# KhutornoyYaroslav/vcm-ts

Measured on AMD Instinct MI355X. Metric: encoded frames/sec at 1920x1080 GOP-32, higher is better.
Workload: dtype f32 (fp16x3 split-MFMA, fp32 accumulate)

## Files before the change

include/dcvc_hip.h:

```cpp
#ifndef DCVC_HIP_H
#define DCVC_HIP_H

#include <stdint.h>

#ifdef __cplusplus
extern "C" {
#endif

#define DCVC_OK 0
#define DCVC_E_ARG (-1)
#define DCVC_E_LAUNCH (-2)
#define DCVC_E_RANGE (-3)

#define DCVC_STATUS_ACT_SATURATED 1

#define DCVC_MAX_SEG 3

#define DCVC_PREC_FP32 0
#define DCVC_PREC_FP16X3 1

typedef struct {
    const float *ptr;
    int32_t C;
    int32_t cs;
} dcvc_seg;

typedef struct {
    dcvc_seg seg[DCVC_MAX_SEG];
    int32_t nseg;
    int32_t N, Hin, Win;
    int32_t in_act;
    float in_slope;
    const float *wpack;
    const float *bpack;
    int32_t ks;
    int32_t stride;
    int32_t Cout;
    int32_t Cout_pad;
    float *out;
    int32_t out_cs;
    int32_t out_act;
    float out_slope;
    int32_t pixel_shuffle;
    const float *res;
    int32_t res_cs;
    const float *res_gate;
    const float *res2;
    int32_t res2_cs;
    int32_t precision;
    int32_t *status;
    float *chan_partial;
    int32_t tile_row0;
    int32_t tile_rows;
    int32_t pair_taps;
} dcvc_conv_args;

int32_t dcvc_conv_tile_rows(int32_t ks, int32_t stride);

int32_t dcvc_conv_chan_partial_parts(int32_t ks, int32_t stride, int32_t Hout, int32_t Wout);
int dcvc_channel_mean_finish(const float *chan_partial, int32_t parts, int32_t row_stride, float *mean, int32_t N,
                             int32_t C, int32_t HW, void *stream);

int64_t dcvc_conv_pack_size(int32_t Cout, int32_t ks, int32_t nseg, const int32_t *seg_C, int32_t *cout_pad);

int dcvc_conv_pack_weights(const float *w, const float *b, int32_t Cout, int32_t ks, int32_t nseg,
                           const int32_t *seg_C, int32_t pixel_shuffle, int32_t precision, float *wpack,
                           float *bpack);

int64_t dcvc_conv_pack_size_paired(int32_t Cout, int32_t Cin, int32_t *cout_pad);
int dcvc_conv_pack_weights_paired(const float *w, const float *b, int32_t Cout, int32_t Cin, float *wpack, float *bpack);

int dcvc_conv2d(const dcvc_conv_args *a, void *stream);

int64_t dcvc_conv_small_pack_bytes(int32_t Cout, int32_t ks, int32_t nseg, const int32_t *seg_C);
int dcvc_conv_small_pack_weights(const float *w, const float *b, int32_t Cout, int32_t ks, int32_t nseg,
                                 const int32_t *seg_C, void *wpack, float *bpack);
int dcvc_conv2d_small(const dcvc_conv_args *a, void *stream);

int64_t dcvc_conv_k32_pack_bytes(int32_t Cout, int32_t ks, int32_t nseg, const int32_t *seg_C, int32_t *cout_pad);
int dcvc_conv_k32_pack_weights(const float *w, const float *b, int32_t Cout, int32_t ks, int32_t nseg,
                               const int32_t *seg_C, int32_t pixel_shuffle, void *wpack, float *bpack);
int dcvc_conv2d_k32(const dcvc_conv_args *a, void *stream);
int dcvc_conv_k32_set_waves(int32_t waves);

int dcvc_warp(const float *src, int32_t src_cs, const float *flow, int32_t flow_cs, float *out, int32_t out_cs,
              int32_t N, int32_t H, int32_t W, int32_t C, void *stream);
int dcvc_up2(const float *src, int32_t src_cs, float *out, int32_t out_cs, float *out2, int32_t out2_cs,
             int32_t N, int32_t H, int32_t W, int32_t C, float scale, void *stream);
int dcvc_down2(const float *src, int32_t src_cs, float *out, int32_t out_cs, int32_t N, int32_t H, int32_t W,
               int32_t C, float scale, int32_t avgpool_order, void *stream);
int dcvc_maxpool2(const float *src, int32_t src_cs, float *out, int32_t out_cs, int32_t N, int32_t H, int32_t W,
                  int32_t C, void *stream);
int dcvc_copy_channels(const float *src, int32_t src_cs, float *out, int32_t out_cs, int64_t npix, int32_t C,
                       void *stream);
int dcvc_nchw_to_nhwc(const float *src, float *out, int32_t out_cs, int32_t N, int32_t C, int32_t H, int32_t W,
                      void *stream);
int dcvc_nhwc_to_nchw(const float *src, int32_t src_cs, float *out, int32_t N, int32_t C, int32_t H, int32_t W,
                      int32_t clamp01, void *stream);

int dcvc_channel_mean(const float *src, int32_t src_cs, float *mean, float *scratch, int32_t N, int32_t HW,
                      int32_t C, void *stream);
int dcvc_se_gate(const float *mean, const float *w1, const float *w2, float *gate, int32_t N, int32_t C,
                 int32_t Cr, void *stream);

int dcvc_scale_channels(const float *src, int32_t src_cs, float *out, int32_t out_cs, const float *q_basic,
                        const float *q_scale, int32_t mode, int32_t N, int32_t HW, int32_t C, void *stream);
int dcvc_round_symbols(const float *z, int32_t z_cs, float *z_hat, int32_t zh_cs, int32_t *sym, int32_t N,
                       int32_t H, int32_t W, int32_t C, void *stream);
int dcvc_symbols_to_nhwc(const int32_t *sym, float *out, int32_t out_cs, int32_t N, int32_t H, int32_t W,
                         int32_t C, void *stream);

typedef struct {
    const float *y;
    int32_t y_cs;
    const float *fusion;
    int32_t fusion_cs;
    const float *spatial;
    int32_t spatial_cs;
    float *params;
    int32_t params_cs;
    float *y_hat;
    float *y_q;
    float *y_res;
    float *scales_hat;
    int32_t *sym;
// ... 36 lines not shown
```

vcm_ts_amd/csrc/conv_mfma.hip:

```cpp
#include <hip/hip_runtime.h>
#include <stdint.h>
#include <stdlib.h>
#include <string.h>
#include <vector>

#include "dcvc_hip.h"

typedef float f32x16 __attribute__((ext_vector_type(16)));
typedef float f32x4 __attribute__((ext_vector_type(4)));
typedef _Float16 f16x8 __attribute__((ext_vector_type(8)));
typedef _Float16 f16x4 __attribute__((ext_vector_type(4)));

namespace {

constexpr int KC = 16;
constexpr int LDK = 20;

constexpr float ACT_SCALE = 8.f;
constexpr float WGT_SCALE = 64.f;
constexpr float F16_MAX = 65504.f;

struct ConvK {
    const float *seg_ptr[DCVC_MAX_SEG];
    int seg_C[DCVC_MAX_SEG];
    int seg_cs[DCVC_MAX_SEG];
    int nseg;
    int Hin, Win, Hout, Wout;
    int in_act;
    float in_slope;
    const float *wpack;
    const float *bpack;
    int Cout, Cout_pad;
    float *out;
    int out_cs;
    int out_act;
    float out_slope;
    int ps;
    const float *res;
    int res_cs;
    const float *res_gate;
    const float *res2;
    int res2_cs;
    int vec_epi;
    int *status;
    float *chan_partial;
    int ntx;
    int ty0, nty;
    int band_rows;
};

constexpr float ACT_LIMIT = 65504.f / 8.f;

__device__ __forceinline__ float act(float v, float slope) { return v > 0.f ? v : v * slope; }

inline long dev_env_long(const char *name, long dflt) {
    const char *dev = getenv("DCVC_DEV");
    if (!dev || strcmp(dev, "1") != 0) return dflt;
    const char *v = getenv(name);
    return v ? atol(v) : dflt;
}


template <int KS, int S, int RPW, int NT, bool SPLIT, bool PAIR = false>
__global__ __launch_bounds__(256, 2) void conv_mfma(const ConvK a) {
    static_assert(!PAIR || (KS == 7 && S == 1 && SPLIT), "tap pairing is built for the 7x7 split-fp16 layers");
    constexpr int BH = 4 * RPW, BW = 32, BN = 32 * NT;
    constexpr int PH = (BH - 1) * S + KS, PW = (BW - 1) * S + KS, PAD = KS / 2;
    constexpr int T = PAIR ? KS * 4 : KS * KS;
    constexpr int TPS = PAIR ? 4 : (KS == 3 && S == 1) ? 9 : KS;
    constexpr int NST = T / TPS;
    constexpr int EPI_LD = BN + 4;
    constexpr int LDS_MAIN = PH * PW * LDK + TPS * 4 * BN * 4, LDS_EPI = 4 * 32 * EPI_LD, LDS_RED = 4 * BN;
    __shared__ __attribute__((aligned(16))) float lds[LDS_MAIN > LDS_EPI + LDS_RED ? LDS_MAIN : LDS_EPI + LDS_RED];
    float *patch = lds;
    float *wl = lds + PH * PW * LDK;

    const int tid = threadIdx.x, lane = tid & 63, wave = tid >> 6;
    const int nbn = a.Cout_pad / BN;
    const int nb = blockIdx.x % nbn, tx = blockIdx.x / nbn;
    if (tx >= a.ntx) return;
    const int ty = blockIdx.y + a.ty0;
    const int x0 = tx * BW, y0 = ty * BH, n0 = nb * BN, img = blockIdx.z;

    f32x16 acc[RPW][NT];
#pragma unroll
    for (int m = 0; m < RPW; ++m)
#pragma unroll
        for (int n = 0; n < NT; ++n)
#pragma unroll
            for (int r = 0; r < 16; ++r) acc[m][n][r] = 0.f;

    const int a_base = ((wave * RPW * S) * PW + (lane & 31) * S) * LDK + (lane >> 5) * 4;
    const int b_base = ((lane >> 5) * BN + (lane & 31)) * 4;

    constexpr int NP = (PH * PW * 4 + 255) / 256, NW = (TPS * 4 * BN + 255) / 256;
    f32x4 rp[NP], rw[NW];
    struct Cursor {
        int s, c0, cg, st;
    };
    auto advance = [&](Cursor &k) {
        if (++k.st == NST) {
            k.st = 0;
            ++k.cg;
            k.c0 += KC;
            if (k.c0 >= a.seg_C[k.s]) {
                ++k.s;
                k.c0 = 0;
            }
        }
    };
    int poff[NP];
    unsigned inpic = 0;
#pragma unroll
    for (int u = 0; u < NP; ++u) {
        const int i = tid + u * 256;
        const int p = i >> 2;
        const int py = p / PW, px = p - py * PW + (PAIR ? (i & 3) >> 1 : 0);
        const int gy = y0 * S - PAD + py, gx = x0 * S - PAD + px;
        const bool ok = i < PH * PW * 4 && gy >= 0 && gy < a.Hin && gx >= 0 && gx < a.Win;
        poff[u] = ok ? gy * a.Win + gx : 0;
        inpic |= (ok ? 1u : 0u) << u;
    }
    auto load_patch = [&](const Cursor &k) {
        const int C = a.seg_C[k.s], cs = a.seg_cs[k.s];
        const float *sp = a.seg_ptr[k.s] + (size_t)img * a.Hin * a.Win * cs;
        const int c = PAIR ? (tid & 1) * 4 : k.c0 + (tid & 3) * 4;
        const int cc = c < C ? c : 0;
#pragma unroll
        for (int u = 0; u < NP; ++u) rp[u] = *(const f32x4 *)(sp + (size_t)poff[u] * cs + cc);
    };
    auto store_patch = [&](const Cursor &k) {
        const int C = a.seg_C[k.s];
#pragma unroll
        for (int u = 0; u < NP; ++u) {
            const int i = tid + u * 256;
            if (i < PH * PW * 4) {
                const int c = PAIR ? (i & 1) * 4 : k.c0 + (i & 3) * 4;
                f32x4 v = ((inpic >> u) & 1u) && c < C ? rp[u] : (f32x4){0.f, 0.f, 0.f, 0.f};
                if (c + 3 >= C) {
                    if (c + 1 >= C) v[1] = 0.f;
                    if (c + 2 >= C) v[2] = 0.f;
                    v[3] = 0.f;
                }
                if (a.in_act) {
                    v[0] = act(v[0], a.in_slope);
                    v[1] = act(v[1], a.in_slope);
                    v[2] = act(v[2], a.in_slope);
                    v[3] = act(v[3], a.in_slope);
                }
                if (!SPLIT) {
                    *(f32x4 *)&patch[(i >> 2) * LDK + (i & 3) * 4] = v;
                } else {
                    f32x4 sv = v * ACT_SCALE;
#pragma unroll
                    for (int e = 0; e < 4; ++e) sv[e] = __builtin_amdgcn_fmed3f(sv[e], -F16_MAX, F16_MAX);
                    const f16x4 hi = __builtin_convertvector(sv, f16x4);
                    const f16x4 lo = __builtin_convertvector(sv - __builtin_convertvector(hi, f32x4), f16x4);
                    _Float16 *rec = (_Float16 *)&patch[(i >> 2) * LDK];
                    *(f16x4 *)&rec[(i & 3) * 4] = hi;
                    *(f16x4 *)&rec[16 + (i & 3) * 4] = lo;
                }
            }
        }
    };
    auto load_w = [&](const Cursor &k) {
        const float *wsrc = a.wpack + ((size_t)(k.cg * T + k.st * TPS) * 4) * a.Cout_pad * 4 + (size_t)n0 * 4;
#pragma unroll
        for (int u = 0; u < NW; ++u) {
            const int i = tid + u * 256;
            const int row = i / BN, col = i - row * BN;
            if (i < TPS * 4 * BN) rw[u] = *(const f32x4 *)(wsrc + ((size_t)row * a.Cout_pad + col) * 4);
        }
    };
    auto store_w = [&]() {
#pragma unroll
        for (int u = 0; u < NW; ++u) {
            const int i = tid + u * 256;
            if (i < TPS * 4 * BN) *(f32x4 *)&wl[i * 4] = rw[u];
        }
    };

    Cursor cur = {0, 0, 0, 0};
    load_patch(cur);
    load_w(cur);
    while (cur.s < a.nseg) {
        __syncthreads();
        if (cur.st == 0) store_patch(cur);
        store_w();
        __syncthreads();
        Cursor nxt = cur;
        advance(nxt);
        if (nxt.s < a.nseg) {
            if (nxt.st == 0) load_patch(nxt);
            load_w(nxt);
        }
        const int a_st = (TPS == T) ? 0 : cur.st * PW * LDK;
#pragma unroll
        for (int tt = 0; tt < TPS; ++tt) {
            const int ky = (TPS == T) ? tt / KS : 0, kx = PAIR ? 2 * tt : (TPS == T) ? tt % KS : tt;
            if (!SPLIT) {
#pragma unroll
                for (int k2 = 0; k2 < 2; ++k2) {
                    f32x4 af[RPW], bf[NT];
#pragma unroll
                    for (int m = 0; m < RPW; ++m)
                        af[m] = *(const f32x4 *)&patch[a_base + a_st + ((m * S + ky) * PW + kx) * LDK + k2 * 8];
#pragma unroll
                    for (int n = 0; n < NT; ++n)
                        bf[n] = *(const f32x4 *)&wl[b_base + ((tt * 4 + k2 * 2) * BN + n * 32) * 4];
#pragma unroll
                    for (int j = 0; j < 4; ++j)
#pragma unroll
                        for (int m = 0; m < RPW; ++m)
#pragma unroll
                            for (int n = 0; n < NT; ++n)
                                acc[m][n] = __builtin_amdgcn_mfma_f32_32x32x2f32(af[m][j], bf[n][j], acc[m][n], 0, 0, 0);
                }
            } else {
                f16x8 ah[RPW], al[RPW], bh[NT], bl[NT];
#pragma unroll
                for (int m = 0; m < RPW; ++m) {
                    const float *rec = &patch[a_base + a_st + ((m * S + ky) * PW + kx) * LDK];
                    ah[m] = *(const f16x8 *)rec;
                    al[m] = *(const f16x8 *)(rec + 8);
                }
#pragma unroll
                for (int n = 0; n < NT; ++n) {
                    bh[n] = *(const f16x8 *)&wl[b_base + ((tt * 4) * BN + n * 32) * 4];
                    bl[n] = *(const f16x8 *)&wl[b_base + ((tt * 4 + 2) * BN + n * 32) * 4];
                }
#pragma unroll
                for (int m = 0; m < RPW; ++m)
#pragma unroll
                    for (int n = 0; n < NT; ++n) {
                        acc[m][n] = __builtin_amdgcn_mfma_f32_32x32x16_f16(ah[m], bh[n], acc[m][n], 0, 0, 0);
                        acc[m][n] = __builtin_amdgcn_mfma_f32_32x32x16_f16(ah[m], bl[n], acc[m][n], 0, 0, 0);
                        acc[m][n] = __builtin_amdgcn_mfma_f32_32x32x16_f16(al[m], bh[n], acc[m][n], 0, 0, 0);
                    }
            }
        }
        cur = nxt;
    }

    const int col = lane & 31, hh = lane >> 5;
    const int Cq = a.Cout >> 2;
    const int Cfin = a.ps ? Cq : a.Cout;
    const int Ho = a.ps ? a.Hout * 2 : a.Hout, Wo = a.ps ? a.Wout * 2 : a.Wout;
    const float inv_scale = SPLIT ? 1.f / (ACT_SCALE * WGT_SCALE) : 1.f;
    float vmax = 0.f;
    if (a.vec_epi) {
        constexpr int LPP = BN / 4, PPI = 64 / LPP, NIT = 32 / PPI;
        float *epi = lds + wave * 32 * EPI_LD;
        const int c4 = (lane % LPP) * 4, pl = lane / LPP;
        const int ch = n0 + c4;
        const bool ch_ok = ch < a.Cout;
        int dy = 0, dx = 0, cf = ch;
        if (a.ps) {
            const int sub = ch / Cq;
            cf = ch - sub * Cq;
            dy = sub >> 1;
            dx = sub & 1;
        }
        f32x4 bias = {0.f, 0.f, 0.f, 0.f}, gate = {1.f, 1.f, 1.f, 1.f};
        if (ch_ok) {
            bias = *(const f32x4 *)&a.bpack[ch];
            if (a.res_gate) gate = *(const f32x4 *)&a.res_gate[(size_t)img * Cfin + cf];
        }
        __syncthreads();
        size_t pix[RPW][NIT];
        bool ok[RPW][NIT];
        f32x4 rv[RPW][NIT], rv2[RPW][NIT];
        f32x4 csum = {0.f, 0.f, 0.f, 0.f};
#pragma unroll
        for (int m = 0; m < RPW; ++m) {
            const int oy = y0 + wave * RPW + m;
#pragma unroll
            for (int it = 0; it < NIT; ++it) {
// ... 69 lines not shown
        return;
    }
#pragma unroll
    for (int m = 0; m < RPW; ++m) {
        const int oy = y0 + wave * RPW + m;
        if (oy >= a.Hout) continue;
#pragma unroll
        for (int n = 0; n < NT; ++n) {
            const int ch = n0 + n * 32 + col;
            if (ch >= a.Cout) continue;
            const float bias = a.bpack[ch];
            int dy = 0, dx = 0, cf = ch;
            if (a.ps) {
                const int sub = ch / Cq;
                cf = ch - sub * Cq;
                dy = sub >> 1;
                dx = sub & 1;
            }
            const float gate = a.res_gate ? a.res_gate[(size_t)img * Cfin + cf] : 1.f;
            float rv[16], rv2[16];
#pragma unroll
            for (int r = 0; r < 16; ++r) {
                const int ox = x0 + (r & 3) + 8 * (r >> 2) + 4 * hh;
                const size_t pix = a.ps ? ((size_t)(img * Ho + 2 * oy + dy) * Wo + 2 * ox + dx)
                                        : ((size_t)(img * Ho + oy) * Wo + ox);
                rv[r] = (a.res && ox < a.Wout) ? a.res[pix * a.res_cs + cf] : 0.f;
                rv2[r] = (a.res2 && ox < a.Wout) ? a.res2[pix * a.res2_cs + cf] : 0.f;
            }
#pragma unroll
            for (int r = 0; r < 16; ++r) {
                const int ox = x0 + (r & 3) + 8 * (r >> 2) + 4 * hh;
                if (ox >= a.Wout) continue;
                float v = acc[m][n][r] * inv_scale + bias;
                if (a.out_act == 1) v = act(v, a.out_slope);
                else if (a.out_act == 2) v = fminf(fmaxf(v, 0.f), 1.f);
                const size_t pix = a.ps ? ((size_t)(img * Ho + 2 * oy + dy) * Wo + 2 * ox + dx)
                                        : ((size_t)(img * Ho + oy) * Wo + ox);
                if (a.out_act == 3) {
                    const float mk = rv2[r] > 0.f ? 1.f : a.out_slope;
                    v = a.res ? __builtin_fmaf(v, mk, rv[r]) : v * mk;
                } else {
                    if (a.res) v = a.res_gate ? __builtin_fmaf(rv[r], gate, v) : v + rv[r];
                    if (a.res2) v = rv2[r] + v;
                }
                if (a.status) vmax = fmaxf(vmax, fabsf(v));
                a.out[pix * a.out_cs + cf] = v;
            }
        }
    }
    if (a.status && !(vmax <= ACT_LIMIT)) atomicOr(a.status, DCVC_STATUS_ACT_SATURATED);
}


template <int KS, int S, int RPW, int NT, bool PAIR = false>
int launch(ConvK &k, int N, hipStream_t st, int precision) {
    constexpr int BH = 4 * RPW, BN = 32 * NT;
    k.ntx = (k.Wout + 31) / 32;
    static const bool xcd_pad = dev_env_long("DCVC_XCD_PAD", 0) != 0;
    unsigned gx = (unsigned)(k.ntx * (k.Cout_pad / BN));
    if (xcd_pad && gx >= 8) gx = (gx + 7) & ~7u;
    k.nty = (k.Hout + BH - 1) / BH;
    if (k.ty0 < 0 || k.ty0 >= k.nty) return DCVC_E_ARG;
    const int rows = k.band_rows > 0 ? (k.band_rows < k.nty - k.ty0 ? k.band_rows : k.nty - k.ty0) : k.nty;
    dim3 grid(gx, (unsigned)rows, (unsigned)N);
    if (PAIR)
        hipLaunchKernelGGL((conv_mfma<KS, S, RPW, NT, true, PAIR>), grid, dim3(256), 0, st, k);
    else if (precision == DCVC_PREC_FP16X3)
        hipLaunchKernelGGL((conv_mfma<KS, S, RPW, NT, true>), grid, dim3(256), 0, st, k);
    else
        hipLaunchKernelGGL((conv_mfma<KS, S, RPW, NT, false>), grid, dim3(256), 0, st, k);
    return hipGetLastError() == hipSuccess ? DCVC_OK : DCVC_E_LAUNCH;
}

inline int round_up(int v, int m) { return (v + m - 1) / m * m; }

}

extern "C" int64_t dcvc_conv_pack_size(int32_t Cout, int32_t ks, int32_t nseg, const int32_t *seg_C, int32_t *cout_pad) {
    if (Cout <= 0 || nseg <= 0 || nseg > DCVC_MAX_SEG || (ks != 1 && ks != 3 && ks != 7)) return DCVC_E_ARG;
    int chunks = 0;
    for (int s = 0; s < nseg; ++s) chunks += (seg_C[s] + KC - 1) / KC;
    const int cp = round_up(Cout, 32);
    if (cout_pad) *cout_pad = cp;
    return (int64_t)chunks * ks * ks * 4 * cp * 4;
}

extern "C" int dcvc_conv_pack_weights(const float *w, const float *b, int32_t Cout, int32_t ks, int32_t nseg,
                                      const int32_t *seg_C, int32_t pixel_shuffle, int32_t precision, float *wpack,
                                      float *bpack) {
    if (precision != DCVC_PREC_FP32 && precision != DCVC_PREC_FP16X3) return DCVC_E_ARG;
    int32_t cp = 0;
    const int64_t total = dcvc_conv_pack_size(Cout, ks, nseg, seg_C, &cp);
    if (total < 0 || (pixel_shuffle && (Cout & 3))) return DCVC_E_ARG;
    const int T = ks * ks;
    int Cin = 0;
    for (int s = 0; s < nseg; ++s) Cin += seg_C[s];
    memset(wpack, 0, (size_t)total * sizeof(float));
    memset(bpack, 0, (size_t)cp * sizeof(float));
    const int Cq = Cout / 4;
    int cg = 0, cin0 = 0;
    for (int s = 0; s < nseg; ++s) {
        for (int c0 = 0; c0 < seg_C[s]; c0 += KC, ++cg) {
            for (int t = 0; t < T; ++t)
                for (int kq = 0; kq < 4; ++kq)
                    for (int j = 0; j < 4; ++j) {
                        const int c = c0 + kq * 4 + j;
                        if (c >= seg_C[s]) continue;
                        for (int n = 0; n < Cout; ++n) {
                            const int np = pixel_shuffle ? (n & 3) * Cq + (n >> 2) : n;
                            const float v = w[((size_t)n * Cin + cin0 + c) * T + t];
                            if (precision == DCVC_PREC_FP32) {
                                wpack[((((size_t)cg * T + t) * 4 + kq) * cp + np) * 4 + j] = v;
                            } else {
                                const int cc = kq * 4 + j, h = cc >> 3, jj = cc & 7;
                                float sv = v * WGT_SCALE;
                                sv = sv > F16_MAX ? F16_MAX : (sv < -F16_MAX ? -F16_MAX : sv);
                                const _Float16 hi = (_Float16)sv, lo = (_Float16)(sv - (float)hi);
                                _Float16 *base = (_Float16 *)wpack;
// ... 6 lines not shown
        cin0 += seg_C[s];
    }
    for (int n = 0; n < Cout; ++n) {
        const int np = pixel_shuffle ? (n & 3) * Cq + (n >> 2) : n;
        bpack[np] = b ? b[n] : 0.f;
    }
    return DCVC_OK;
}

extern "C" int64_t dcvc_conv_pack_size_paired(int32_t Cout, int32_t Cin, int32_t *cout_pad) {
    if (Cout <= 0 || Cin <= 0 || Cin > 8) return DCVC_E_ARG;
    const int cp = round_up(Cout, 32);
    if (cout_pad) *cout_pad = cp;
    return (int64_t)7 * 4 * 4 * cp * 4;
}

extern "C" int dcvc_conv_pack_weights_paired(const float *w, const float *b, int32_t Cout, int32_t Cin, float *wpack, float *bpack) {
    int32_t cp = 0;
    const int64_t total = dcvc_conv_pack_size_paired(Cout, Cin, &cp);
    if (total < 0 || !w || !wpack || !bpack) return DCVC_E_ARG;
    memset(wpack, 0, (size_t)total * sizeof(float));
    memset(bpack, 0, (size_t)cp * sizeof(float));
    _Float16 *base = (_Float16 *)wpack;
    bool clamped = false;
    for (int ky = 0; ky < 7; ++ky)
        for (int kx = 0; kx < 7; ++kx) {
            const int step = ky * 4 + (kx >> 1), h = kx & 1;
            for (int c = 0; c < Cin; ++c)
                for (int n = 0; n < Cout; ++n) {
                    float sv = w[((size_t)n * Cin + c) * 49 + ky * 7 + kx] * WGT_SCALE;
                    if (!(fabsf(sv) <= F16_MAX)) {
                        clamped = true;
                        sv = sv > 0.f ? F16_MAX : -F16_MAX;
                    }
                    const _Float16 hi = (_Float16)sv, lo = (_Float16)(sv - (float)hi);
                    base[(((size_t)step * 4 + h) * cp + n) * 8 + c] = hi;
                    base[(((size_t)step * 4 + 2 + h) * cp + n) * 8 + c] = lo;
                }
        }
    for (int n = 0; n < Cout; ++n) bpack[n] = b ? b[n] : 0.f;
    return clamped ? DCVC_E_RANGE : DCVC_OK;
}

static int tile_rows(int ks, int stride) { return stride == 2 ? 4 : 8; }

extern "C" int32_t dcvc_conv_tile_rows(int32_t ks, int32_t stride) { return tile_rows(ks, stride); }

extern "C" int32_t dcvc_conv_chan_partial_parts(int32_t ks, int32_t stride, int32_t Hout, int32_t Wout) {
    if (Hout <= 0 || Wout <= 0 || (stride != 1 && stride != 2)) return DCVC_E_ARG;
    const int bh = tile_rows(ks, stride);
    return ((Wout + 31) / 32) * ((Hout + bh - 1) / bh);
}

extern "C" int dcvc_conv2d(const dcvc_conv_args *a, void *stream) {
    if (!a || a->nseg < 1 || a->nseg > DCVC_MAX_SEG || !a->out || !a->wpack || !a->bpack) return DCVC_E_ARG;
    if (a->stride != 1 && a->stride != 2) return DCVC_E_ARG;
    if (a->precision != DCVC_PREC_FP32 && a->precision != DCVC_PREC_FP16X3) return DCVC_E_ARG;
    if (a->Cout_pad % 32 || a->Cout > a->Cout_pad || (a->pixel_shuffle && (a->Cout & 3))) return DCVC_E_ARG;
    if (a->out_act < 0 || a->out_act > 3) return DCVC_E_ARG;
    if (a->out_act == 3 && (!a->res2 || a->res_gate || a->chan_partial || a->pixel_shuffle)) return DCVC_E_ARG;
    ConvK k;
    memset(&k, 0, sizeof(k));
    for (int s = 0; s < a->nseg; ++s) {
        if (!a->seg[s].ptr || (a->seg[s].cs & 3) || a->seg[s].cs < round_up(a->seg[s].C, 4) ||
            ((uintptr_t)a->seg[s].ptr & 15))
            return DCVC_E_ARG;
        k.seg_ptr[s] = a->seg[s].ptr;
        k.seg_C[s] = a->seg[s].C;
        k.seg_cs[s] = a->seg[s].cs;
    }
    k.nseg = a->nseg;
    k.Hin = a->Hin;
    k.Win = a->Win;
    const int pad = a->ks / 2;
    k.Hout = (a->Hin + 2 * pad - a->ks) / a->stride + 1;
    k.Wout = (a->Win + 2 * pad - a->ks) / a->stride + 1;
    k.in_act = a->in_act;
    k.in_slope = a->in_slope;
    k.wpack = a->wpack;
    k.bpack = a->bpack;
    k.Cout = a->Cout;
    k.Cout_pad = a->Cout_pad;
    k.out = a->out;
    k.out_cs = a->out_cs;
    k.out_act = a->out_act;
    k.out_slope = a->out_slope;
    k.ps = a->pixel_shuffle;
    k.res = a->res;
    k.res_cs = a->res_cs;
    k.res_gate = a->res_gate;
    k.res2 = a->res2;
    k.res2_cs = a->res2_cs;
    k.status = a->status;
    k.chan_partial = a->chan_partial;
    k.ty0 = a->tile_rows > 0 ? a->tile_row0 : 0;
    k.band_rows = a->tile_rows > 0 ? a->tile_rows : 0;
    {
        const int cfin = a->pixel_shuffle ? a->Cout / 4 : a->Cout;
        auto al = [](const void *p, int cs) { return p == nullptr || ((((uintptr_t)p) & 15) == 0 && (cs & 3) == 0); };
        k.vec_epi = (cfin % 4 == 0) && al(a->out, a->out_cs) && al(a->res, a->res_cs) && al(a->res2, a->res2_cs) &&
                    (a->res_gate == nullptr || (((uintptr_t)a->res_gate) & 15) == 0);
    }
    if (a->chan_partial && (!k.vec_epi || a->pixel_shuffle)) return DCVC_E_ARG;
    hipStream_t st = (hipStream_t)stream;
    const bool wide = (a->Cout_pad % 64) == 0;
    const int key = a->ks * 10 + a->stride;
    if (a->stride == 1 && !a->pair_taps && !a->chan_partial && a->tile_rows <= 0) {
        const long wgs8 = (long)((k.Wout + 31) / 32) * ((k.Hout + 7) / 8) * (a->Cout_pad / (wide ? 64 : 32)) * a->N;
        static const long rows4_below = dev_env_long("DCVC_ROWS4_WGS", 384);
        if (wgs8 < rows4_below) {
            if (a->ks == 3) return wide ? launch<3, 1, 1, 2>(k, a->N, st, a->precision) : launch<3, 1, 1, 1>(k, a->N, st, a->precision);
            if (a->ks == 7) return wide ? launch<7, 1, 1, 2>(k, a->N, st, a->precision) : launch<7, 1, 1, 1>(k, a->N, st, a->precision);
            if (a->ks == 1) return wide ? launch<1, 1, 1, 2>(k, a->N, st, a->precision) : launch<1, 1, 1, 1>(k, a->N, st, a->precision);
        }
    }
    switch (key) {
        case 11: return wide ? launch<1, 1, 2, 2>(k, a->N, st, a->precision) : launch<1, 1, 2, 1>(k, a->N, st, a->precision);
        case 12: return wide ? launch<1, 2, 1, 2>(k, a->N, st, a->precision) : launch<1, 2, 1, 1>(k, a->N, st, a->precision);
        case 31:
            return wide ? launch<3, 1, 2, 2>(k, a->N, st, a->precision) : launch<3, 1, 2, 1>(k, a->N, st, a->precision);
        case 32: return wide ? launch<3, 2, 1, 2>(k, a->N, st, a->precision) : launch<3, 2, 1, 1>(k, a->N, st, a->precision);
        case 71:
            if (a->pair_taps) {
                if (a->nseg != 1 || a->seg[0].C > 8 || a->precision != DCVC_PREC_FP16X3 || a->pixel_shuffle) return DCVC_E_ARG;
                return wide ? launch<7, 1, 2, 2, true>(k, a->N, st, a->precision) : launch<7, 1, 2, 1, true>(k, a->N, st, a->precision);
            }
            return wide ? launch<7, 1, 2, 2>(k, a->N, st, a->precision) : launch<7, 1, 2, 1>(k, a->N, st, a->precision);
        default: return DCVC_E_ARG;
    }
}
```

vcm_ts_amd/engine.py:

```python
from __future__ import annotations

import ctypes as C
import math

import numpy as np
import torch

from . import lib

_raw_stream = getattr(torch._C, "_cuda_getCurrentRawStream", None) or (lambda idx: torch.cuda.current_stream(idx).cuda_stream)


def _r4(c):
    return (c + 3) // 4 * 4


class View:

    __slots__ = ("base", "N", "H", "W", "C", "cs", "coff", "ptr")

    def __init__(self, base: torch.Tensor, C_: int, coff: int = 0, geom=None):
        self.base = base
        if geom is None:
            assert base.dim() == 4 and base.dtype == torch.float32 and base.is_contiguous()
# ... 17 lines not shown
        return None

    def slice(self, c0: int, c: int) -> "View":
        v = View(self.base, c, 0, geom=(self.N, self.H, self.W, self.cs, self.ptr + 4 * c0))
        v.coff = self.coff + c0
        return v

    def nchw(self) -> torch.Tensor:
        if self.base.dim() == 4 and tuple(self.base.shape) == (self.N, self.H, self.W, self.cs):
            return self.base[..., self.coff : self.coff + self.C].permute(0, 3, 1, 2)
        return self.base[:, self.coff : self.coff + self.C]

    @property
    def HW(self):
        return self.H * self.W

    def __repr__(self):
        return f"View(N={self.N},H={self.H},W={self.W},C={self.C},cs={self.cs},coff={self.coff})"


class PackedConv:
    __slots__ = ("w", "b", "ks", "Cout", "Cout_pad", "seg_C", "ps", "version", "precision", "weight", "bias",
                 "cin_slice", "key", "small", "k32", "paired", "host", "job")


class Engine:
    def __init__(self, device, precision=None):
        import os

        self.precision = precision or os.environ.get("DCVC_PRECISION", "fp32")
        if self.precision not in lib.PRECISIONS:
            raise ValueError(f"precision must be one of {sorted(lib.PRECISIONS)}")
        self.device = torch.device(device)
        if self.device.type != "cuda":
            raise RuntimeError("the HIP engine needs a GPU device (no CPU fallback exists)")
        self._dev_index = self.device.index if self.device.index is not None else torch.cuda.current_device()
        self.L = lib.hip()
        self.bufs = {}
        self.packs = {}
        self._dev_packs = []
        self._plan = None
        self.calls = 0
        self.profile = None
        self.profile_detail = None
        self.profile_hbm = None
        self.tape = None
        self._edges = {}
        self._status = None
        dev = os.environ.get("DCVC_DEV") == "1"
        sw = lambda name, default: os.environ.get(name, default) if dev else default
        self.use_small = sw("DCVC_SMALL", "1") != "0"
        self.use_k32 = sw("DCVC_K32", "1") != "0"
        self.use_pairs = sw("DCVC_PAIR_TAPS", "1") != "0"
        self.k32_everywhere = False
        self.k32_sizes = tuple(int(k) for k in sw("DCVC_K32_SIZES", "3").split(","))
        self.range_check = os.environ.get("DCVC_RANGE_CHECK", "1") == "1"
        self.guard_outputs = True
        self.wgrad_split = os.environ.get("DCVC_WGRAD_SPLIT", "1") != "0"
        self.wgrad_side_stream = sw("DCVC_WGRAD_SIDE", "1") != "0"

    def stream(self):
        return C.c_void_p(_raw_stream(self._dev_index))

    def _store(self, scratch=False):
        return self.bufs if (self.tape is None or scratch) else self.tape.arena

    def buf(self, name, N, H, W, C_, cs=None, zero=False) -> View:
        cs = cs or _r4(C_)
        key = (name, N, H, W, cs)
        store = self._store()
        t = store.get(key)
        if t is None:
            t = (torch.zeros if zero else torch.empty)((N, H, W, cs), dtype=torch.float32, device=self.device)
            store[key] = t
        return View(t, C_)

    def status_word(self) -> torch.Tensor:
        if self._status is None:
            self._status = torch.zeros(1, dtype=torch.int32, device=self.device)
        return self._status

    def read_status(self) -> int:
        if self._status is None:
            return 0
        v = int(self._status.item())
        if v:
            self._status.zero_()
        return v

    def check_status(self):
        v = self.read_status()
        if v:
            raise lib.KernelError(f"split-fp16 activation range exceeded (status {v}): |x| > 8188; use precision='fp32'")

    def status_snapshot(self):
        if self._status is None:
            return None
        host = torch.empty(1, dtype=torch.int32, pin_memory=True)
        host.copy_(self._status, non_blocking=True)
        ev = torch.cuda.Event()
        ev.record(torch.cuda.current_stream(self.device))

        def check():
            ev.synchronize()
            v = int(host[0])
            if v:
# ... 226 lines not shown
        q.ks, q.Cout, q.Cout_pad, q.seg_C, q.ps, q.version, q.key = pk.ks, pk.Cout, cpad.value, pk.seg_C, False, pk.version, pk.key
        pk.paired = q
        return q

    def pair_capable(self, pk: PackedConv, stride) -> bool:
        return (self.precision == "fp16x3" and self.tape is None and self.use_pairs and getattr(pk, "host", False)
                and pk.ks == 7 and stride == 1 and len(pk.seg_C) == 1 and pk.seg_C[0] <= 8 and not pk.ps and pk.Cout > 16)

    def pack_k32(self, pk: PackedConv) -> PackedConv:
        q = getattr(pk, "k32", None)
        if q is not None and q.version == pk.version:
            return q
        w = pk.weight.detach().float().cpu()
        if pk.cin_slice is not None:
            w = w[:, pk.cin_slice[0] : pk.cin_slice[1]]
        w = w.contiguous().numpy()
        b = None if pk.bias is None else pk.bias.detach().float().cpu().contiguous().numpy()
        segs = (C.c_int32 * len(pk.seg_C))(*pk.seg_C)
        cpad = C.c_int32()
        n = self.L.dcvc_conv_k32_pack_bytes(pk.Cout, pk.ks, len(pk.seg_C), segs, C.byref(cpad))
        if n < 0:
            raise lib.KernelError(f"conv_k32_pack_bytes({pk.key})")
        wp = np.empty(n // 4, np.float32)
        bp = np.empty(cpad.value, np.float32)
        lib.check(self.L.dcvc_conv_k32_pack_weights(w.ctypes.data, None if b is None else b.ctypes.data, pk.Cout, pk.ks,
                                                    len(pk.seg_C), segs, int(pk.ps), wp.ctypes.data, bp.ctypes.data),
                  f"conv_k32_pack_weights({pk.key}) [status -3: a |weight| >= 1023.5 does not fit split fp16, use precision='fp32']")
        q = PackedConv()
        q.w, q.b = torch.from_numpy(wp).to(self.device), torch.from_numpy(bp).to(self.device)
        q.ks, q.Cout, q.Cout_pad, q.seg_C, q.ps, q.version, q.key = pk.ks, pk.Cout, cpad.value, pk.seg_C, pk.ps, pk.version, pk.key
        pk.k32 = q
        return q

    def k32_capable(self, pk: PackedConv, stride, out: View, res, res2, gate, srcs=()) -> bool:
        if not (self.precision == "fp16x3" and self.tape is None and self.use_k32 and getattr(pk, "host", False)):
            return False
        cfin = pk.Cout // 4 if pk.ps else pk.Cout
        al = lambda v: v is None or (v.ptr % 16 == 0 and v.cs % 4 == 0)
        covered = (pk.ks in self.k32_sizes and stride == 1 and all(c % 32 == 0 for c in pk.seg_C) and cfin % 4 == 0
                   and al(out) and al(res) and al(res2) and (gate is None or gate.data_ptr() % 16 == 0)
                   and all(al(s) for s in srcs) and out.H * out.W < (1 << 24)
                   and all(v is None or v.cs * 4 < (1 << 24) for v in (out, res, res2, *srcs)))
        if not covered or self.k32_everywhere:
            return covered
        m = 2 if pk.ps else 1
        tiles = ((out.H // m + 7) // 8) * ((out.W // m + 31) // 32)
        return pk.Cout_pad % 64 == 0 and tiles * (pk.Cout_pad // 64) >= 1000

    def small_capable(self, pk: PackedConv, stride, gate, res2, chan_partial) -> bool:
        return (self.precision == "fp16x3" and self.tape is None and self.use_small and getattr(pk, "host", False)
                and pk.Cout <= 16 and pk.ks in (3, 7)
                and stride == 1 and not pk.ps and gate is None and res2 is None and chan_partial is None)

    def conv(self, pk: PackedConv, srcs, out: View, stride=1, in_slope=None, out_slope=None, res: View = None,
             gate: torch.Tensor = None, res2: View = None, chan_partial: torch.Tensor = None, band=None):
        return self._conv_f32(pk, srcs, out, stride, in_slope, out_slope, res, gate, res2, chan_partial, band)

    def _launch_conv(self, launch, pk, s0, Ho, Wo, stride, res, res2, tag="", note=""):
        if self.profile is None:
            launch()
            return
        ev0, ev1 = torch.cuda.Event(enable_timing=True), torch.cuda.Event(enable_timing=True)
        ev0.record()
        launch()
        ev1.record()
        flops = 2.0 * s0.N * Ho * Wo * pk.Cout * sum(pk.seg_C) * pk.ks * pk.ks
        nout = s0.N * Ho * Wo * pk.Cout
        abytes = 4.0 * (s0.N * s0.H * s0.W * sum(pk.seg_C) + nout * (1 + (res is not None) + (res2 is not None))
                        + pk.Cout * sum(pk.seg_C) * pk.ks * pk.ks)
        self.profile.setdefault(f"conv{pk.ks}x{pk.ks}s{stride}{tag}", []).append((ev0, ev1, flops, abytes))
        if self.profile_detail is not None:
            self.profile_detail.append((ev0, ev1, flops, f"k{pk.ks}s{stride}{tag} {pk.seg_C}->{pk.Cout}{'ps' if pk.ps else ''} "
                                                         f"{s0.H}x{s0.W}", note))

    def chan_partial_buf(self, name, pk: PackedConv, out: View, stride=1):
        parts = int(self.L.dcvc_conv_chan_partial_parts(pk.ks, stride, out.H, out.W))
        if parts <= 0:
            raise lib.KernelError("conv_chan_partial_parts")
        return self.fbuf(name + ".chan_partial", out.N * parts * pk.Cout_pad), parts

    def _conv_f32(self, pk: PackedConv, srcs, out: View, stride=1, in_slope=None, out_slope=None, res: View = None,
                  gate: torch.Tensor = None, res2: View = None, chan_partial: torch.Tensor = None, band=None):
        a = lib.ConvArgs()
        assert len(srcs) == len(pk.seg_C)
        s0 = srcs[0]
        for i, (s, c) in enumerate(zip(srcs, pk.seg_C)):
            assert s.C == c and (s.N, s.H, s.W) == (s0.N, s0.H, s0.W), (s, c)
            a.seg[i].ptr, a.seg[i].C, a.seg[i].cs = s.ptr, s.C, s.cs
        a.nseg, a.N, a.Hin, a.Win = len(srcs), s0.N, s0.H, s0.W
        a.in_act, a.in_slope = (0, 0.0) if in_slope is None else (1, in_slope)
        small = band is None and self.small_capable(pk, stride, gate, res2, chan_partial)
        k32 = not small and not isinstance(out_slope, tuple) and self.k32_capable(pk, stride, out, res, res2, gate, srcs)
        paired = not small and not k32 and self.pair_capable(pk, stride)
        wq = self.pack_small(pk) if small else (self.pack_k32(pk) if k32 else (self.pack_paired(pk) if paired else pk))
        a.pair_taps = int(paired)
        a.wpack, a.bpack = wq.w.data_ptr(), wq.b.data_ptr()
        a.ks, a.stride, a.Cout, a.Cout_pad = pk.ks, stride, pk.Cout, wq.Cout_pad
        pad = pk.ks // 2
        Ho = (s0.H + 2 * pad - pk.ks) // stride + 1
        Wo = (s0.W + 2 * pad - pk.ks) // stride + 1
        m = 2 if pk.ps else 1
        cfin = pk.Cout // 4 if pk.ps else pk.Cout
        assert (out.N, out.H, out.W, out.C) == (s0.N, Ho * m, Wo * m, cfin), (out, Ho, Wo, cfin)
        a.out, a.out_cs = out.ptr, out.cs
        if isinstance(out_slope, tuple):
            assert out_slope[0] == "mask" and res2 is not None and not (small or k32)
            a.out_act, a.out_slope = 3, float(out_slope[1])
        else:
            a.out_act, a.out_slope = (0, 0.0) if out_slope is None else ((2, 0.0) if out_slope == "clamp01" else (1, out_slope))
        a.pixel_shuffle = int(pk.ps)
        a.precision = pk.precision
        if res is not None:
            assert (res.N, res.H, res.W, res.C) == (out.N, out.H, out.W, out.C)
            a.res, a.res_cs = res.ptr, res.cs
        if gate is not None:
            a.res_gate = gate.data_ptr()
        if res2 is not None:
            assert (res2.N, res2.H, res2.W, res2.C) == (out.N, out.H, out.W, out.C)
            a.res2, a.res2_cs = res2.ptr, res2.cs
        if (self.range_check or k32) and self.precision == "fp16x3" and self.guard_outputs:
            a.status = self.status_word().data_ptr()
        if chan_partial is not None:
            a.chan_partial = chan_partial.data_ptr()
        if band is not None:
            a.tile_row0, a.tile_rows = int(band[0]), int(band[1])
        fn, what = (self.L.dcvc_conv2d_small, "conv2d_small") if small else (
            (self.L.dcvc_conv2d_k32, "conv2d_k32") if k32 else (self.L.dcvc_conv2d, "conv2d"))
        note = ""
        if self.profile_detail is not None:
            note = (f"{pk.key[0][1] if isinstance(pk.key[0], tuple) and len(pk.key[0]) > 1 else pk.key[0]}"
                    f" in_act={in_slope} out_act={out_slope} in_cs={[s.cs for s in srcs]} out_cs={out.cs}"
                    f" res={None if res is None else res.cs} gate={gate is not None} res2={None if res2 is None else res2.cs}"
                    f" chan_sums={chan_partial is not None}")
        self._launch_conv(lambda: lib.check(fn(C.byref(a), self.stream()), what), pk, s0, Ho, Wo, stride, res, res2,
                          "small" if small else ("k32" if k32 else ""), note)
        self.calls += 1
        self._rec("conv", pk, tuple(srcs), out, stride, in_slope, out_slope, res, gate, res2)
        return out

    def _hbm(self, kernel, shape, abytes, launch):
        if self.profile_hbm is None:
            return launch()
        ev0, ev1 = torch.cuda.Event(enable_timing=True), torch.cuda.Event(enable_timing=True)
        ev0.record()
        launch()
        ev1.record()
        self.profile_hbm.setdefault((kernel, shape), []).append((ev0, ev1, float(abytes)))

    def collect_profile_hbm(self):
        torch.cuda.synchronize(self.device)
        out = []
        for (kernel, shape), v in (self.profile_hbm or {}).items():
            ms = sum(r[0].elapsed_time(r[1]) for r in v)
            by = sum(r[2] for r in v)
            out.append({"kernel": kernel, "shape": shape, "launches": len(v), "avg_us": round(ms / len(v) * 1e3, 2),
                        "algorithmic_bytes": int(by / len(v)), "tb_per_s": round(by / (ms * 1e-3) / 1e12, 3) if ms > 0 else None})
        return out

    def collect_profile(self):
        torch.cuda.synchronize(self.device)
        return {k: {"flops": sum(r[2] for r in v), "bytes": sum(r[3] for r in v),
                    "ms": sum(r[0].elapsed_time(r[1]) for r in v), "launches": len(v)}
                for k, v in (self.profile or {}).items()}

    def warp(self, src: View, flow: View, out: View):
        self._hbm("warp", f"C{src.C} {src.H}x{src.W}", src.N * src.H * src.W * (8 * src.C + 8),
                  lambda: lib.check(self.L.dcvc_warp(src.ptr, src.cs, flow.ptr, flow.cs, out.ptr, out.cs, src.N, src.H, src.W,
                                                     src.C, self.stream()), "warp"))
        self.calls += 1
        self._rec("warp", src, flow, out)
        return out

    def up2(self, src: View, out: View, scale=1.0, out2: View = None):
        n_in = src.N * src.H * src.W * src.C * 4
        self._hbm("up2", f"C{src.C} {src.H}x{src.W}", n_in * (1 + 4 * (2 if out2 else 1)),
                  lambda: lib.check(self.L.dcvc_up2(src.ptr, src.cs, out.ptr, out.cs, out2.ptr if out2 else None,
                                                    out2.cs if out2 else 0, src.N, src.H, src.W, src.C, scale, self.stream()), "up2"))
        self.calls += 1
        self._rec("up2", src, out, scale, out2)
        return out

    def down2(self, src: View, out: View, scale=1.0, avgpool_order=False):
        self._hbm("down2", f"C{src.C} {src.H}x{src.W}", src.N * src.H * src.W * src.C * 5,
                  lambda: lib.check(self.L.dcvc_down2(src.ptr, src.cs, out.ptr, out.cs, src.N, src.H, src.W, src.C, scale,
                                                      int(avgpool_order), self.stream()), "down2"))
        self.calls += 1
        self._rec_unary("down2", src, out, scale)
        return out
# ... 129 lines not shown
```

vcm_ts_amd/lib.py:

```python
from __future__ import annotations

import ctypes as C
import os

HERE = os.path.dirname(os.path.abspath(__file__))
CSRC = os.path.join(HERE, "csrc")


class LibraryMissing(RuntimeError):
    pass


class KernelError(RuntimeError):
    pass


def _load(name):
    path = os.environ.get("DCVC_HIP_LIB") if name == "libdcvc_hip.so" and os.environ.get("DCVC_HIP_LIB") else \
        os.path.join(CSRC, name)
    if not os.path.exists(path):
        raise LibraryMissing(f"{path} not built; run `make -C {CSRC}` (no CPU fallback exists)")
    return C.CDLL(path)


# ... 49 lines not shown
        ("C", C.c_int32), ("step", C.c_int32), ("idx_edges", C.c_void_p), ("forced_q", C.c_void_p),
    ]


class ConvBwdArgs(C.Structure):
    _fields_ = [
        ("dout", C.c_void_p), ("dout_cs", C.c_int32), ("out", C.c_void_p), ("out_cs", C.c_int32),
        ("res", C.c_void_p), ("res_cs", C.c_int32), ("gate", C.c_void_p), ("res2", C.c_void_p), ("res2_cs", C.c_int32),
        ("dres", C.c_void_p), ("dres_cs", C.c_int32), ("dres2", C.c_void_p), ("dres2_cs", C.c_int32),
        ("dpre", C.c_void_p), ("dpre_cs", C.c_int32), ("zs", C.c_int32), ("Hd", C.c_int32), ("Wd", C.c_int32),
        ("N", C.c_int32), ("Ho", C.c_int32), ("Wo", C.c_int32), ("Cout", C.c_int32), ("pixel_shuffle", C.c_int32),
        ("act", C.c_int32), ("slope", C.c_float),
    ]


class WgradArgs(C.Structure):
    _fields_ = [
        ("x", C.c_void_p), ("x_cs", C.c_int32), ("C", C.c_int32), ("in_act", C.c_int32), ("in_slope", C.c_float),
        ("dpre", C.c_void_p), ("dpre_cs", C.c_int32), ("zs", C.c_int32), ("Hd", C.c_int32), ("Wd", C.c_int32),
        ("N", C.c_int32), ("Hin", C.c_int32), ("Win", C.c_int32), ("Ho", C.c_int32), ("Wo", C.c_int32),
        ("Cout", C.c_int32), ("ks", C.c_int32), ("stride", C.c_int32), ("dw", C.c_void_p), ("Cin_total", C.c_int32),
        ("cin_offset", C.c_int32), ("scratch", C.c_void_p), ("scratch_floats", C.c_int64), ("overwrite", C.c_int32),
        ("db", C.c_void_p), ("precision", C.c_int32),
    ]


class PackJob(C.Structure):
    _fields_ = [
        ("w", C.c_void_p), ("b", C.c_void_p), ("Cout", C.c_int32), ("Cin_total", C.c_int32), ("ks", C.c_int32),
        ("nseg", C.c_int32), ("seg_C", C.c_int32 * 3), ("cin_offset", C.c_int32), ("pixel_shuffle", C.c_int32),
        ("precision", C.c_int32), ("transposed", C.c_int32), ("wpack", C.c_void_p), ("bpack", C.c_void_p),
    ]


class DualPriorBwdArgs(C.Structure):
    _fields_ = [
        ("y", C.c_void_p), ("y_cs", C.c_int32), ("fusion", C.c_void_p), ("fusion_cs", C.c_int32),
        ("y_hat", C.c_void_p), ("dout", C.c_void_p), ("dout_cs", C.c_int32), ("dy_res", C.c_void_p),
        ("dscales_hat", C.c_void_p), ("dparams", C.c_void_p), ("dparams_cs", C.c_int32),
        ("dspatial", C.c_void_p), ("dspatial_cs", C.c_int32), ("dy", C.c_void_p), ("dy_cs", C.c_int32),
        ("dfusion", C.c_void_p), ("dfusion_cs", C.c_int32), ("dq_plane", C.c_void_p),
        ("q_basic", C.c_void_p), ("q_scale", C.c_void_p), ("N", C.c_int32), ("H", C.c_int32), ("W", C.c_int32),
        ("C", C.c_int32), ("step", C.c_int32),
    ]


PRECISIONS = {"fp32": 0, "fp16x3": 1}

_hip = None
i32, i64, f32, vp = C.c_int32, C.c_int64, C.c_float, C.c_void_p

_SIGS = {
    "dcvc_conv2d": [C.POINTER(ConvArgs), vp],
    "dcvc_conv_pack_weights": [vp, vp, i32, i32, i32, vp, i32, i32, vp, vp],
    "dcvc_conv_pack_weights_paired": [vp, vp, i32, i32, vp, vp],
    "dcvc_conv2d_small": [C.POINTER(ConvArgs), vp],
    "dcvc_conv_small_pack_weights": [vp, vp, i32, i32, i32, vp, vp, vp],
    "dcvc_conv2d_k32": [C.POINTER(ConvArgs), vp],
    "dcvc_conv_k32_pack_weights": [vp, vp, i32, i32, i32, vp, i32, vp, vp],
    "dcvc_conv_k32_set_waves": [i32],
    "dcvc_warp": [vp, i32, vp, i32, vp, i32, i32, i32, i32, i32, vp],
    "dcvc_up2": [vp, i32, vp, i32, vp, i32, i32, i32, i32, i32, f32, vp],
    "dcvc_down2": [vp, i32, vp, i32, i32, i32, i32, i32, f32, i32, vp],
    "dcvc_maxpool2": [vp, i32, vp, i32, i32, i32, i32, i32, vp],
    "dcvc_copy_channels": [vp, i32, vp, i32, i64, i32, vp],
    "dcvc_nchw_to_nhwc": [vp, vp, i32, i32, i32, i32, i32, vp],
    "dcvc_nhwc_to_nchw": [vp, i32, vp, i32, i32, i32, i32, i32, vp],
    "dcvc_channel_mean": [vp, i32, vp, vp, i32, i32, i32, vp],
    "dcvc_se_gate": [vp, vp, vp, vp, i32, i32, i32, vp],
    "dcvc_channel_mean_finish": [vp, i32, i32, vp, i32, i32, i32, vp],
    "dcvc_scale_channels": [vp, i32, vp, i32, vp, vp, i32, i32, i32, i32, vp],
    "dcvc_round_symbols": [vp, i32, vp, i32, vp, i32, i32, i32, i32, vp],
    "dcvc_symbols_to_nhwc": [vp, vp, i32, i32, i32, i32, i32, vp],
    "dcvc_scale_indexes": [vp, vp, i64, vp, vp],
    "dcvc_dual_prior_enc": [C.POINTER(DualPriorArgs), vp],
    "dcvc_dual_prior_dec_index": [C.POINTER(DualPriorArgs), vp],
    "dcvc_dual_prior_dec_apply": [C.POINTER(DualPriorArgs), vp],
    "dcvc_build_scale_cdfs": [vp, i32, i32, vp, vp, vp, vp],
    "dcvc_build_factorized_cdfs": [vp, i32, vp, vp, vp, vp],
    "dcvc_scale_bits": [vp, vp, vp, vp, i32, i32, i64, vp],
    "dcvc_factorized_bits": [vp, i32, vp, vp, vp, i32, i32, i32, vp],
    "dcvc_sq_err": [vp, i32, vp, i32, vp, vp, i32, i32, i32, vp],
    "dcvc_conv_pack_weights_dev": [vp, vp, i32, i32, i32, i32, vp, i32, i32, i32, i32, vp, vp, vp],
    "dcvc_pack_plan_create": [C.POINTER(PackJob), i32, C.POINTER(C.c_void_p)],
    "dcvc_pack_plan_run": [vp, vp],
    "dcvc_pack_plan_destroy": [vp],
    "dcvc_conv_bwd_prologue": [C.POINTER(ConvBwdArgs), vp],
    "dcvc_conv_wgrad": [C.POINTER(WgradArgs), vp],
    "dcvc_channel_dot": [vp, i32, vp, i32, vp, vp, i32, i32, i32, i32, i32, vp],
    "dcvc_mask_accumulate": [vp, i32, vp, i32, f32, vp, i32, i64, i32, vp],
    "dcvc_add_planes": [vp, i32, vp, i32, vp, i32, i64, i32, vp],
    "dcvc_warp_bwd": [vp, i32, vp, i32, vp, i32, vp, i32, vp, i32, i32, i32, i32, i32, vp, vp],
    "dcvc_up2_bwd": [vp, i32, vp, i32, i32, i32, i32, i32, f32, vp],
    "dcvc_down2_bwd": [vp, i32, vp, i32, i32, i32, i32, i32, f32, vp],
    "dcvc_maxpool2_bwd": [vp, i32, vp, i32, vp, i32, i32, i32, i32, i32, vp],
    "dcvc_se_bwd": [vp, vp, vp, vp, vp, vp, vp, vp, i32, i32, i32, vp],
    "dcvc_add_channel_vec": [vp, i32, vp, f32, i32, i32, i32, vp],
    "dcvc_scale_channels_bwd": [vp, i32, vp, i32, vp, vp, i32, i32, i32, i32, vp],
    "dcvc_q_finish": [vp, vp, vp, vp, vp, vp, i32, i32, vp],
    "dcvc_dual_prior_bwd": [C.POINTER(DualPriorBwdArgs), vp],
    "dcvc_scale_bits_bwd": [vp, vp, vp, vp, vp, i32, i32, i64, vp],
    "dcvc_factorized_bits_bwd": [vp, i32, vp, vp, vp, i32, vp, i32, i32, i32, vp],
    "dcvc_sq_err_bwd": [vp, i32, vp, i32, vp, vp, i32, i32, i32, i32, vp],
    "dcvc_drans_encode": [vp, vp, i32, i32, i64, vp, i32, i32, vp, vp, i32, vp, i64, vp, i64, vp, vp, vp, vp],
    "dcvc_drans_decode": [vp, i64, vp, vp, vp, i32, i32, i64, vp, i32, i32, vp, vp, vp, i32, vp, vp, vp],
    "dcvc_drans_build_lut": [vp, i32, i32, vp, vp],
# ... 50 lines not shown
```

Baseline: 42.07.

## Add planar even/odd-column LDS patch layout for 3x3 stride-2 split-fp16 convs

Adds a PLANAR variant of the MFMA conv kernel for 3x3 stride-2 fp16x3 layers. It stores the input patch in LDS with even and odd columns split into separate planes, as 64-byte records with an XOR swizzle, so the strided A-fragment reads of adjacent lanes hit contiguous, bank-spread addresses. The goal is to remove LDS bank conflicts from stride-2 access; it also drops the LDK padding, which shrinks patch LDS. A new entry point dcvc_conv2d_s2 and engine routing (DCVC_S2, on by default) select it.

```diff
diff --git a/include/dcvc_hip.h b/include/dcvc_hip.h
--- a/include/dcvc_hip.h
+++ b/include/dcvc_hip.h
@@ -71,6 +71,8 @@
 int dcvc_conv_pack_weights_paired(const float *w, const float *b, int32_t Cout, int32_t Cin, float *wpack, float *bpack);
 
 int dcvc_conv2d(const dcvc_conv_args *a, void *stream);
+
+int dcvc_conv2d_s2(const dcvc_conv_args *a, void *stream);
 
 int64_t dcvc_conv_small_pack_bytes(int32_t Cout, int32_t ks, int32_t nseg, const int32_t *seg_C);
 int dcvc_conv_small_pack_weights(const float *w, const float *b, int32_t Cout, int32_t ks, int32_t nseg,
diff --git a/vcm_ts_amd/csrc/conv_mfma.hip b/vcm_ts_amd/csrc/conv_mfma.hip
--- a/vcm_ts_amd/csrc/conv_mfma.hip
+++ b/vcm_ts_amd/csrc/conv_mfma.hip
@@ -61,19 +61,22 @@
 }
 
 
-template <int KS, int S, int RPW, int NT, bool SPLIT, bool PAIR = false>
+template <int KS, int S, int RPW, int NT, bool SPLIT, bool PAIR = false, bool PLANAR = false>
 __global__ __launch_bounds__(256, 2) void conv_mfma(const ConvK a) {
     static_assert(!PAIR || (KS == 7 && S == 1 && SPLIT), "tap pairing is built for the 7x7 split-fp16 layers");
+    static_assert(!PLANAR || (KS == 3 && S == 2 && SPLIT && !PAIR), "the planar patch is built for 3x3 stride-2 split-fp16 layers");
     constexpr int BH = 4 * RPW, BW = 32, BN = 32 * NT;
     constexpr int PH = (BH - 1) * S + KS, PW = (BW - 1) * S + KS, PAD = KS / 2;
+    constexpr int PW0 = (PW + 1) / 2;
+    constexpr int REC = PLANAR ? 16 : LDK;
     constexpr int T = PAIR ? KS * 4 : KS * KS;
-    constexpr int TPS = PAIR ? 4 : (KS == 3 && S == 1) ? 9 : KS;
+    constexpr int TPS = PAIR ? 4 : ((KS == 3 && S == 1) || PLANAR) ? 9 : KS;
     constexpr int NST = T / TPS;
     constexpr int EPI_LD = BN + 4;
-    constexpr int LDS_MAIN = PH * PW * LDK + TPS * 4 * BN * 4, LDS_EPI = 4 * 32 * EPI_LD, LDS_RED = 4 * BN;
+    constexpr int LDS_MAIN = PH * PW * REC + TPS * 4 * BN * 4, LDS_EPI = 4 * 32 * EPI_LD, LDS_RED = 4 * BN;
     __shared__ __attribute__((aligned(16))) float lds[LDS_MAIN > LDS_EPI + LDS_RED ? LDS_MAIN : LDS_EPI + LDS_RED];
     float *patch = lds;
-    float *wl = lds + PH * PW * LDK;
+    float *wl = lds + PH * PW * REC;
 
     const int tid = threadIdx.x, lane = tid & 63, wave = tid >> 6;
     const int nbn = a.Cout_pad / BN;
@@ -156,9 +159,18 @@
                     for (int e = 0; e < 4; ++e) sv[e] = __builtin_amdgcn_fmed3f(sv[e], -F16_MAX, F16_MAX);
                     const f16x4 hi = __builtin_convertvector(sv, f16x4);
                     const f16x4 lo = __builtin_convertvector(sv - __builtin_convertvector(hi, f32x4), f16x4);
-                    _Float16 *rec = (_Float16 *)&patch[(i >> 2) * LDK];
-                    *(f16x4 *)&rec[(i & 3) * 4] = hi;
-                    *(f16x4 *)&rec[16 + (i & 3) * 4] = lo;
+                    if (PLANAR) {
+                        const int p = i >> 2, py = p / PW, px = p - py * PW;
+                        const int q = py * PW + ((px & 1) ? PW0 + (px >> 1) : (px >> 1));
+                        const int sw = (q >> 2) & 3, h = (i & 3) >> 1;
+                        char *rec = (char *)patch + q * 64 + (i & 1) * 8;
+                        *(f16x4 *)(rec + ((h ^ sw) << 4)) = hi;
+                        *(f16x4 *)(rec + (((2 + h) ^ sw) << 4)) = lo;
+                    } else {
+                        _Float16 *rec = (_Float16 *)&patch[(i >> 2) * LDK];
+                        *(f16x4 *)&rec[(i & 3) * 4] = hi;
+                        *(f16x4 *)&rec[16 + (i & 3) * 4] = lo;
+                    }
                 }
             }
         }
@@ -220,9 +232,17 @@
                 f16x8 ah[RPW], al[RPW], bh[NT], bl[NT];
 #pragma unroll
                 for (int m = 0; m < RPW; ++m) {
-                    const float *rec = &patch[a_base + a_st + ((m * S + ky) * PW + kx) * LDK];
-                    ah[m] = *(const f16x8 *)rec;
-                    al[m] = *(const f16x8 *)(rec + 8);
+                    if (PLANAR) {
+                        const int q = ((wave * RPW + m) * S + ky) * PW + ((kx & 1) ? PW0 : (kx >> 1)) + (lane & 31);
+                        const char *rec = (const char *)patch + q * 64;
+                        const int sl = ((lane >> 5) ^ ((q >> 2) & 3)) << 4;
+                        ah[m] = *(const f16x8 *)(rec + sl);
+                        al[m] = *(const f16x8 *)(rec + (sl ^ 32));
+                    } else {
+                        const float *rec = &patch[a_base + a_st + ((m * S + ky) * PW + kx) * LDK];
+                        ah[m] = *(const f16x8 *)rec;
+                        al[m] = *(const f16x8 *)(rec + 8);
+                    }
                 }
 #pragma unroll
                 for (int n = 0; n < NT; ++n) {
@@ -398,7 +418,7 @@
 }
 
 
-template <int KS, int S, int RPW, int NT, bool PAIR = false>
+template <int KS, int S, int RPW, int NT, bool PAIR = false, bool PLANAR = false>
 int launch(ConvK &k, int N, hipStream_t st, int precision) {
     constexpr int BH = 4 * RPW, BN = 32 * NT;
     k.ntx = (k.Wout + 31) / 32;
@@ -409,7 +429,9 @@
     if (k.ty0 < 0 || k.ty0 >= k.nty) return DCVC_E_ARG;
     const int rows = k.band_rows > 0 ? (k.band_rows < k.nty - k.ty0 ? k.band_rows : k.nty - k.ty0) : k.nty;
     dim3 grid(gx, (unsigned)rows, (unsigned)N);
-    if (PAIR)
+    if constexpr (PLANAR)
+        hipLaunchKernelGGL((conv_mfma<KS, S, RPW, NT, true, false, true>), grid, dim3(256), 0, st, k);
+    else if (PAIR)
         hipLaunchKernelGGL((conv_mfma<KS, S, RPW, NT, true, PAIR>), grid, dim3(256), 0, st, k);
     else if (precision == DCVC_PREC_FP16X3)
         hipLaunchKernelGGL((conv_mfma<KS, S, RPW, NT, true>), grid, dim3(256), 0, st, k);
@@ -522,7 +544,7 @@
     return ((Wout + 31) / 32) * ((Hout + bh - 1) / bh);
 }
 
-extern "C" int dcvc_conv2d(const dcvc_conv_args *a, void *stream) {
+static int conv2d(const dcvc_conv_args *a, void *stream, bool planar) {
     if (!a || a->nseg < 1 || a->nseg > DCVC_MAX_SEG || !a->out || !a->wpack || !a->bpack) return DCVC_E_ARG;
     if (a->stride != 1 && a->stride != 2) return DCVC_E_ARG;
     if (a->precision != DCVC_PREC_FP32 && a->precision != DCVC_PREC_FP16X3) return DCVC_E_ARG;
@@ -589,7 +611,9 @@
         case 12: return wide ? launch<1, 2, 1, 2>(k, a->N, st, a->precision) : launch<1, 2, 1, 1>(k, a->N, st, a->precision);
         case 31:
             return wide ? launch<3, 1, 2, 2>(k, a->N, st, a->precision) : launch<3, 1, 2, 1>(k, a->N, st, a->precision);
-        case 32: return wide ? launch<3, 2, 1, 2>(k, a->N, st, a->precision) : launch<3, 2, 1, 1>(k, a->N, st, a->precision);
+        case 32:
+            if (planar) return wide ? launch<3, 2, 1, 2, false, true>(k, a->N, st, a->precision) : launch<3, 2, 1, 1, false, true>(k, a->N, st, a->precision);
+            return wide ? launch<3, 2, 1, 2>(k, a->N, st, a->precision) : launch<3, 2, 1, 1>(k, a->N, st, a->precision);
         case 71:
             if (a->pair_taps) {
                 if (a->nseg != 1 || a->seg[0].C > 8 || a->precision != DCVC_PREC_FP16X3 || a->pixel_shuffle) return DCVC_E_ARG;
@@ -599,3 +623,10 @@
         default: return DCVC_E_ARG;
     }
 }
+
+extern "C" int dcvc_conv2d(const dcvc_conv_args *a, void *stream) { return conv2d(a, stream, false); }
+
+extern "C" int dcvc_conv2d_s2(const dcvc_conv_args *a, void *stream) {
+    if (!a || a->ks != 3 || a->stride != 2 || a->precision != DCVC_PREC_FP16X3 || a->pair_taps) return DCVC_E_ARG;
+    return conv2d(a, stream, true);
+}
diff --git a/vcm_ts_amd/engine.py b/vcm_ts_amd/engine.py
--- a/vcm_ts_amd/engine.py
+++ b/vcm_ts_amd/engine.py
@@ -93,6 +93,8 @@
         self.use_small = sw("DCVC_SMALL", "1") != "0"
         self.use_k32 = sw("DCVC_K32", "1") != "0"
         self.use_pairs = sw("DCVC_PAIR_TAPS", "1") != "0"
+        self.use_s2 = sw("DCVC_S2", "1") != "0"
+        self.last_conv = None
         self.k32_everywhere = False
         self.k32_sizes = tuple(int(k) for k in sw("DCVC_K32_SIZES", "3").split(","))
         self.range_check = os.environ.get("DCVC_RANGE_CHECK", "1") == "1"
@@ -425,6 +427,10 @@
                 and pk.Cout <= 16 and pk.ks in (3, 7)
                 and stride == 1 and not pk.ps and gate is None and res2 is None and chan_partial is None)
 
+    def s2_capable(self, pk: PackedConv, stride) -> bool:
+        return (self.precision == "fp16x3" and self.tape is None and self.use_s2 and pk.ks == 3 and stride == 2
+                and pk.precision == lib.PRECISIONS["fp16x3"])
+
     def conv(self, pk: PackedConv, srcs, out: View, stride=1, in_slope=None, out_slope=None, res: View = None,
              gate: torch.Tensor = None, res2: View = None, chan_partial: torch.Tensor = None, band=None):
         return self._conv_f32(pk, srcs, out, stride, in_slope, out_slope, res, gate, res2, chan_partial, band)
@@ -465,6 +471,7 @@
         small = band is None and self.small_capable(pk, stride, gate, res2, chan_partial)
         k32 = not small and not isinstance(out_slope, tuple) and self.k32_capable(pk, stride, out, res, res2, gate, srcs)
         paired = not small and not k32 and self.pair_capable(pk, stride)
+        s2 = not small and not k32 and not paired and self.s2_capable(pk, stride)
         wq = self.pack_small(pk) if small else (self.pack_k32(pk) if k32 else (self.pack_paired(pk) if paired else pk))
         a.pair_taps = int(paired)
         a.wpack, a.bpack = wq.w.data_ptr(), wq.b.data_ptr()
@@ -498,7 +505,9 @@
         if band is not None:
             a.tile_row0, a.tile_rows = int(band[0]), int(band[1])
         fn, what = (self.L.dcvc_conv2d_small, "conv2d_small") if small else (
-            (self.L.dcvc_conv2d_k32, "conv2d_k32") if k32 else (self.L.dcvc_conv2d, "conv2d"))
+            (self.L.dcvc_conv2d_k32, "conv2d_k32") if k32 else (
+                (self.L.dcvc_conv2d_s2, "conv2d_s2") if s2 else (self.L.dcvc_conv2d, "conv2d")))
+        self.last_conv = what
         note = ""
         if self.profile_detail is not None:
             note = (f"{pk.key[0][1] if isinstance(pk.key[0], tuple) and len(pk.key[0]) > 1 else pk.key[0]}"
@@ -506,7 +515,7 @@
                     f" res={None if res is None else res.cs} gate={gate is not None} res2={None if res2 is None else res2.cs}"
                     f" chan_sums={chan_partial is not None}")
         self._launch_conv(lambda: lib.check(fn(C.byref(a), self.stream()), what), pk, s0, Ho, Wo, stride, res, res2,
-                          "small" if small else ("k32" if k32 else ""), note)
+                          "small" if small else ("k32" if k32 else ("planar" if s2 else "")), note)
         self.calls += 1
         self._rec("conv", pk, tuple(srcs), out, stride, in_slope, out_slope, res, gate, res2)
         return out
diff --git a/vcm_ts_amd/lib.py b/vcm_ts_amd/lib.py
--- a/vcm_ts_amd/lib.py
+++ b/vcm_ts_amd/lib.py
@@ -125,6 +125,7 @@
 
 _SIGS = {
     "dcvc_conv2d": [C.POINTER(ConvArgs), vp],
+    "dcvc_conv2d_s2": [C.POINTER(ConvArgs), vp],
     "dcvc_conv_pack_weights": [vp, vp, i32, i32, i32, vp, i32, i32, vp, vp],
     "dcvc_conv_pack_weights_paired": [vp, vp, i32, i32, vp, vp],
     "dcvc_conv2d_small": [C.POINTER(ConvArgs), vp],
```

Result: no change. 42.27 (median of 6 runs) (+0.5%).
